# OSU-NLP-Group/saev

Hardware: AMD Instinct MI355X
Metric: activations/sec (train step), d_in=1024 x32 k=32 (higher is better)
Workload: dtype f32 (encoder: fp16 MFMA first pass with a rigorous error margin, survivors recomputed exactly in fp32; all else fp32)

## Files before the change

### saev_amd/csrc/ctx.hip

```cpp
#include <hip/hip_runtime.h>

#include <algorithm>
#include <cmath>
#include <cstdio>
#include <cstdlib>
#include <cstring>
#include <dlfcn.h>
#include <mutex>
#include <string>
#include <vector>

#include "kernels.h"

namespace {
constexpr int AUX_KSPLIT_MAX = 16;
constexpr int CAND_CAP = 4096;
constexpr int CAND_STRIDE = CAND_CAP + 256;
constexpr int TIMING_RING = 512;
constexpr int DEAD_LAG = 4;
constexpr int DEAD_RING = 16;
enum { AUX_NONE = 0, AUX_SMALL_DEVICE = 1, AUX_SMALL_HOST = 2, AUX_DENSE = 3 };
}

struct saev_ctx {
// ... 54 lines not shown
    bool dws_ok = false;
    int dws_rows = 0;
    bool dws_pairs = false;
    float *gS = nullptr, *xS = nullptr, *dvp = nullptr;
    float* xS_ov = nullptr;
    float* xS_bwd = nullptr;
    float* dval_rows = nullptr;
    bool dval_fwd = false;
    float* wn2 = nullptr;
    float* sq_wave = nullptr;
    int sq_wave_n = 0;
    bool wn2_fresh = false;
    float* WdS = nullptr;
    double* dec_part = nullptr;
    bool wds_fresh = false;
    bool dval_pairs_ready = false;
    bool fused_forward = false;
    bool fwd_slices = false;
    bool fwd_step = false;
    float* rs_part = nullptr;
    float* xS_c = nullptr;
    int2 *pv = nullptr, *pv2 = nullptr;
    int32_t *plat = nullptr, *cut_lat = nullptr, *cut_list = nullptr;
    int32_t* lat_unused = nullptr;
    bool fused_step = false;
    bool unused_valid = false;
    int P = 1;
    int32_t cuts[MAX_PREFIXES] = {0};
    float* G = nullptr;
    float* GS = nullptr;
    int P_cap = 0;
    int n_dead_host = 0, k_use_host = 0;
    int64_t tokens_seen = 0;
    bool tracker_dirty = false;
    int nd_cap = 0;
    DeadRecord* rec_host = nullptr;
    DeadRecord* rec_dev = nullptr;
    hipEvent_t dead_ev[DEAD_RING];
    bool dead_ev_created = false;
    int64_t dead_steps = 0;
    int64_t rec_valid_from = 1;
    int aux_route = AUX_NONE;
    int64_t n_readbacks = 0;
    std::vector<void*> aux_allocs;
    int32_t* dead_list = nullptr;
    float *Wenc_dead = nullptr, *Wdec_dead = nullptr, *H_dead = nullptr, *A_dead = nullptr, *dWd = nullptr, *dWe = nullptr,
// ... 231 lines not shown
    A(chunk_starts, S + 1); A(part_starts, S); A(work_latent, c->max_work);
    A(dW_encT, S * D); A(partials, (size_t)c->max_part * 2 * D); A(db_partials, c->max_part); A(row_proj, S); A(enc_sq, S);
    {
        const bool rows_only = c->dbg.dw_route == 1;
        c->dws_ok = !rows_only && D % DWS_SLICE == 0 && (uint64_t)S * D * 4ull < (1ull << 32) && MBB < (1l << 24) &&
                    (uint64_t)MBB * K < (1ull << 31);
    }
    c->fwd_slices = c->cfg.encoder_mode == SAEV_ENCODER_F16R && (c->dbg.fwd_route == 0 || c->dbg.fwd_route == 2) && c->dbg.fused_chain == 0 && D % RS_SLICE == 0 &&
                    (uint64_t)S * 128ull < (1ull << 32) - 256ull && fused_supported(c->cfg);
    if (c->fwd_slices) {
        A(rs_part, (size_t)(D / RS_SLICE) * MB * REFINE_CAP); A(surv_rng, MB * RS_MAX_RANGES);
        c->rs_lat_range = (int)std::max<long>(RS_LAT_RANGE, ((S + RS_MAX_RANGES - 1) / RS_MAX_RANGES + 255) / 256 * 256);
        c->rs_n_ranges = (int)((S + c->rs_lat_range - 1) / c->rs_lat_range);
    }
    if (c->fwd_slices && !c->dws_ok) A(xS, MBB * D);
    if (c->dws_ok) {
        A(gS, MBB * D); A(xS, MBB * D); A(dvp, (size_t)(D / DWS_SLICE) * MBB * K);
        if (c->dbg.dw_route != 2 && decode_forms_dval((int)D, (int)K)) A(dval_rows, MB * K);
        if (c->dval_rows != nullptr && c->dbg.dw_route == 4 && decode_slices_supported((int)D, (int)S, (int)K, (int)K) && c->cfg.normalize_w_dec) {
            A(WdS, S * D); A(dec_part, (size_t)(D / 32) * MB * 3);
        }
        A(pv, MBB * K); A(pv2, MBB * K); A(plat, MBB * K); A(cut_lat, (MBB * K + DWS_RUN - 1) / DWS_RUN); A(cut_list, 4 * (1 + (MBB * K + DWS_RUN - 1) / DWS_RUN)); A(lat_unused, S);
        if (c->dval_rows != nullptr && c->dbg.fin_route == 0) { A(wn2, S); A(sq_wave, (size_t)2 * dw_slices_waves((int)D, (int)(MBB * K))); }
    }
    A(colsum_partials, ((MBB + 63) / 64) * D);
    A(sumsq_partials, 2 * 1024 + (S + 3) / 4 + 8 + transpose_blocks((int)S, (int)D)); A(sumsq_total, 1);
    if (c->cfg.encoder_mode != SAEV_ENCODER_F32 || KA > 0) {
        c->Dp = (int)((D + 31) / 32 * 32);
        c->S_pad = (int)((S + 255) / 256 * 256);
        c->MB_pad = (int)((MB + 255) / 256 * 256);
        A(zero_bias, std::max(S, D)); A(aux_scales, 16); A(aux_sync, absmax_parts_max((int)MB));
    }
    if (c->cfg.encoder_mode != SAEV_ENCODER_F32) {
        A(xs, (size_t)c->MB_pad * 2 * c->Dp);
        A(ws, (size_t)c->S_pad * 2 * c->Dp);
        A(row_margin, MB); A(wnorm_scratch, std::max((S + 3) / 4, 3 * ((S + 255) / 256))); A(f16r_scales, 16); A(mu, D); A(xnorm, 2 * MB); A(b_shift, S);
        A(xabs_part, (MB + 3) / 4);
        if (c->cfg.encoder_mode == SAEV_ENCODER_F16R) { A(dot_part, (size_t)2 * (c->Dp / 32) * c->S_pad); A(sq_part, (size_t)2 * (c->Dp / 32) * c->S_pad); A(wmax_prev, 1); }
        if (c->cfg.encoder_mode == SAEV_ENCODER_F16R) { A(surv_idx, MB * REFINE_CAP); A(surv_val, MB * REFINE_CAP); A(surv_cnt, MB); }
    }
    c->stream_ok = c->fwd_slices && c->cfg.bound_mode == 0 && c->dbg.prep_route == 0 && D % 32 == 0 && c->Dp == (int)D;
    if (c->stream_ok) {
        A(WeS, S * D); A(xn_part, (size_t)(D / 32) * c->MB_pad * 2);
        A(amax_part, (size_t)(c->MB_pad / 256) * (D / 32)); A(cmax_part, (size_t)(c->MB_pad / 256) * (D / 32)); A(b_seen, S);
        A(mu_keep, D); A(xside_keep, 4);
    }
// ... 756 lines not shown
            HIPCHK(c, launch_normalize_rows(c->params + c->off_W_dec, S, D, s, c->WdS, c->wn2));
            c->wds_fresh = true;
            c->wn2_fresh = c->wn2 != nullptr;
        } else if (c->cfg.normalize_w_dec) {
            HIPCHK(c, launch_normalize_rows(c->params + c->off_W_dec, S, D, s, nullptr, c->wn2));
            c->wn2_fresh = c->wn2 != nullptr;
        }
    }

    DecodeArgs a{};
    a.x = x; a.idx = c->idx; a.val = c->val; a.code_stride = K; a.k = K;
    a.W_dec = c->params + c->off_W_dec; a.b_dec = c->params + c->off_b_dec;
    a.n_rows = n; a.D = D; a.S = S; a.idx_limit = S;
    a.upper = c->upper_c;
    a.gscale = 2.0f / ((float)n * (float)D * (float)c->P);
    a.training = training ? 1 : 0;
    a.g = c->g; a.x_hat = c->x_hat; a.fired = c->fired; a.rowstats = c->rowstats;
    c->dws_rows = 0;
    c->dval_fwd = false;
    if (training && c->dws_ok && (c->P == 1 || c->GS != nullptr)) { a.gS = c->P == 1 ? c->gS : c->GS; a.xS = c->fwd_step ? nullptr : c->xS; c->dws_rows = n; }
    if (c->dws_rows == n && c->dval_rows != nullptr && (c->P == 1 || decode_matry_forms_dval(D, K))) { a.dval_out = c->dval_rows; c->dval_fwd = true; }
    c->bitmap_prefill_words = 0;
    const bool slices_decode = c->P == 1 && c->wds_fresh && a.dval_out != nullptr && a.gS != nullptr;
    if (training && c->dbg.csc_route == 0 && c->bitmap != nullptr && c->bitmap_clean && !c->last_backward_gathered && !slices_decode) {
        const int words = ((n + 31) / 32 + 7) / 8 * 8;
        if (words <= c->bitmap_clean_words) {
            a.csc_bitmap = c->bitmap; a.csc_words = words;
            c->bitmap_prefill_words = words; c->bitmap_prefill_rows = n;
            c->bitmap_clean = false;
        }
    }
    if (slices_decode) {
        DecodeSliceArgs ds{};
        ds.d = a; ds.WdS = c->WdS; ds.part = c->dec_part; ds.dvp = c->dvp; ds.dvp_pitch = (long)c->back_rows * K;
        HIPCHK(c, launch_decode_slices(ds, s));
    } else if (c->P > 1) {
        MatryArgs m{};
        m.P = c->P;
        for (int p = 0; p < c->P; ++p) m.cuts[p] = c->cuts[p];
        m.G = c->G;
        m.g_rows_all = c->fused_forward ? 0 : 1;
        HIPCHK(c, launch_decode_matry(a, m, s));
    } else {
        HIPCHK(c, launch_decode(a, s));
    }
    c->P_last = c->P;
    for (int p = 0; p < c->P; ++p) c->cuts_last[p] = c->cuts[p];
// ... 389 lines not shown
    c->dws_pairs = ov ? ov_slices : c->dws_rows == n;
    if (ov_slices) {
        c->xS_bwd = c->xS;
        if (!c->followers.empty()) {
            if (c->xS_ov == nullptr) {
                int rca = alloc(c, &c->xS_ov, (size_t)c->back_rows * D);
                if (rca != SAEV_OK) return rca;
            }
            c->xS_bwd = c->xS_ov;
        }
        HIPCHK(c, launch_slice_major_copy(c->ov_g, c->ov_x, n, D, c->gS, c->xS_bwd, s));
        c->dws_rows = 0;
    }
    c->csc_epoch = c->csc_epoch == 0x7fffffff ? 1 : c->csc_epoch + 1;
    a.epoch = c->dbg.csc_route == 2 ? 0 : c->csc_epoch;
    if (c->dws_pairs) {
        a.zero_word = c->cut_list;
        a.pv = c->pv; a.plat = c->plat; a.val = ov ? c->ov_val : c->val;
        a.P = c->P_last;
        for (int p = 0; p < c->P_last; ++p) a.cuts[p] = c->cuts_last[p];
        if (!ov && c->dval_fwd) { a.pv2 = c->pv2; a.dval = c->dval_rows; }
    }
    c->dval_pairs_ready = c->dws_pairs && a.pv2 != nullptr;
    if (c->fused_step && c->dws_pairs) { a.pairs = nullptr; a.chunk_starts = nullptr; a.part_starts = nullptr; a.work_latent = nullptr; }
    const float* gmat = ov ? c->ov_g : (c->P_last > 1 ? c->G : c->g);
    const bool prefilled = !ov && c->bitmap_prefill_words == words && c->bitmap_prefill_rows == n;
    HIPCHK(c, launch_csc_build(a, s, c->bitmap_clean && words <= c->bitmap_clean_words, gmat, D, (long)c->P_last * D,
                               c->colsum_partials, c->grads + c->off_b_dec, prefilled));
    c->bitmap_prefill_words = 0;
    c->last_backward_gathered = ov;
    c->bitmap_clean = false;
    c->bitmap_words_last = words;
    if (c->aux_route != AUX_NONE) {
        int rc = auxk_backward(c, s);
        if (rc != SAEV_OK) return rc;
    }
    return SAEV_OK;
}

int saev_backward_rows(saev_ctx* c, int32_t lat_lo, int32_t lat_hi, void* stream) {
    return saev_backward_rows_part(c, lat_lo, lat_hi, 0, stream);
}

int saev_backward_rows_part(saev_ctx* c, int32_t lat_lo, int32_t lat_hi, int32_t part, void* stream) {
    if (!c) return SAEV_INVALID_ARG;
    REQUIRE(c, part >= 0 && part <= 2, SAEV_INVALID_ARG, "saev_backward_rows_part: part must be 0 (both), 1 (decoder) or 2 (encoder)");
// ... 15 lines not shown
    a.partials = c->partials; a.db_partials = c->db_partials;
    a.lat_lo = lat_lo; a.lat_hi = lat_hi;
    a.part = part; a.dval = c->dval_pairs;
    const bool all_rows = part == 0 && lat_lo == 0 && lat_hi == S;
    const bool clears = part != 2 && lat_lo == 0 && lat_hi == S && c->bitmap_words_last > 0;
    if (clears) { a.clear_bitmap = c->bitmap; a.clear_words = c->bitmap_words_last; }
    a.row_proj = all_rows ? c->row_proj : nullptr; a.project = c->cfg.remove_parallel_grads ? 1 : 0;
    a.enc_sq = all_rows ? c->enc_sq : nullptr;
    const int max_work = (lat_hi - lat_lo) + (int)(((long)n * K + DW_CHUNK - 1) / DW_CHUNK);
    if (lat_lo == 0 && lat_hi == S && c->dws_pairs && (ov || c->dws_rows == n)) {
        DwSlicesArgs w{};
        w.starts = c->starts; w.pv = c->pv; w.pv2 = c->pv2; w.plat = c->plat; w.gS = c->P_last > 1 ? c->GS : c->gS; w.W_dec = a.W_dec; w.P = c->P_last;
        w.xS = ov ? c->xS_bwd : (c->fwd_step ? c->xS_c : c->xS);
        w.n_rows = n; w.D = D; w.S = S; w.pair_cap = (int)((long)c->back_rows * K);
        w.dvp = c->dvp; w.dW_dec = a.dW_dec; w.dW_encT = a.dW_encT; w.db_enc = a.db_enc;
        const size_t runs_cap = ((size_t)w.pair_cap + DWS_RUN - 1) / DWS_RUN;
        w.part_dec = c->partials; w.part_enc = c->partials + 2 * runs_cap * D;
        w.cut_lat = c->cut_lat; w.cut_list = c->cut_list;
        w.lat_unused = (all_rows && c->fused_step) ? c->lat_unused : nullptr;
        c->unused_valid = w.lat_unused != nullptr;
        w.row_proj = a.row_proj; w.project = a.project; w.enc_sq = a.enc_sq;
        w.clear_bitmap = a.clear_bitmap; w.clear_words = a.clear_words;
        w.have_dval = c->dval_pairs_ready ? 1 : 0;
        c->sq_wave_n = 0;
        if (c->dval_pairs_ready && c->wn2_fresh && part == 0) {
            w.wn2 = c->wn2;
            if (c->fused_step && all_rows && c->sq_wave != nullptr && c->dbg.fin_route != 2) {
                c->sq_wave_n = dw_slices_waves(D, (int)((long)n * K));
                w.sq_wave_dec = c->sq_wave; w.sq_wave_enc = c->sq_wave + c->sq_wave_n;
            }
        }
        HIPCHK(c, launch_dw_slices(w, (int)((long)n * K), part, s));
    } else {
        c->unused_valid = false;
        HIPCHK(c, launch_dw_rows(a, max_work, s));
    }
    if (c->aux_route == AUX_DENSE)
        HIPCHK(c, launch_scatter_add_dead(c->dead_list, c->n_dead_host, D, c->dWd, c->dWe, c->dbe, c->grads + c->off_W_dec,
                                          c->dW_encT, c->grads + c->off_b_enc, lat_lo, lat_hi, s,
                                          c->aux_dev_count ? c->flags + 4 : nullptr, part, a.row_proj, a.W_dec, a.project, a.enc_sq,
                                          c->unused_valid ? c->lat_unused : nullptr, c->sq_wave_n > 0 ? c->starts : nullptr));
    else if (c->aux_route != AUX_NONE)
        HIPCHK(c, launch_scatter_add_dead(c->dead_list, c->aux_mfma ? c->aux_ndp : AUX_SMALL_MAX, D, c->dWd, c->dWe, c->dbe, c->grads + c->off_W_dec,
                                          c->dW_encT, c->grads + c->off_b_enc, lat_lo, lat_hi, s, c->flags + 4, part,
                                          a.row_proj, a.W_dec, a.project, a.enc_sq, c->unused_valid ? c->lat_unused : nullptr,
                                          c->sq_wave_n > 0 ? c->starts : nullptr));
// ... 540 lines not shown
```

### saev_amd/csrc/kernels.h

```cpp
#pragma once
#include <hip/hip_runtime.h>
#include <stdint.h>

#include "../../include/saev_amd.h"

enum { EPI_DENSE = 0, EPI_TOPK = 1 };

struct EncodeArgs {
    const float* x;
    const float* W_enc;
    const float* b_enc;
    int n_rows, D, S;
    int s_splits;
    float* h_out;
    int ngroups;
    int32_t* gmax;
    int gmax_stride;
    int32_t* cand_cnt;
    float* cand_val;
    int32_t* cand_idx;
    int cand_cap;
    int cand_stride;
    const int32_t* enable_flag;
    int enable_when;
// ... 139 lines not shown

struct CscArgs {
    const int32_t* idx;
    int code_stride, k;
    const int32_t* k_dev;
    int n_rows, S;
    uint32_t* bitmap;
    int words;
    int32_t* grp_prefix;
    int32_t* counts;
    int32_t* scan_totals;
    int32_t* starts;
    int2* pairs;
    int32_t* chunk_starts;
    int32_t* part_starts;
    int32_t* work_latent;
    int2* pv;
    int32_t* plat;
    const float* val;
    int2* pv2;
    const float* dval;
    int P;
    int32_t cuts[16];
    int32_t* zero_word;
    int32_t epoch;
};
hipError_t launch_csc_build(const CscArgs& a, hipStream_t stream, bool bitmap_clean = false, const float* colsum_m = nullptr,
                            int colsum_D = 0, long colsum_row_stride = 0, float* colsum_partials = nullptr,
                            float* colsum_out = nullptr, bool prefilled = false);

constexpr int DW_CHUNK = 64;

struct DwRowsArgs {
    const int32_t* starts;
    const int32_t* chunk_starts;
    const int32_t* work_latent;
    const int32_t* part_starts;
    const int2* pairs;
    const float* val;
    const float* W_dec;
    const float* g;
    const float* x;
    int D, S;
    int P;
    int32_t cuts[MAX_PREFIXES];
    const int32_t* k_dev;
// ... 24 lines not shown
    const float* gS;
    const float* xS;
    const float* W_dec;
    int n_rows, D, S, pair_cap;
    int P;
    float* dvp;
    float* dW_dec;
    float* dW_encT;
    float* db_enc;
    float* part_dec;
    float* part_enc;
    int32_t* cut_lat;
    int32_t* cut_list;
    float2* row_proj;
    int project;
    float* enc_sq;
    uint32_t* clear_bitmap;
    int clear_words;
    int32_t* lat_unused;
    int have_dval;
    const float* wn2;
    float* sq_wave_dec;
    float* sq_wave_enc;
};
hipError_t launch_dw_slices(const DwSlicesArgs& a, int max_pairs, int part, hipStream_t stream);
int dw_slices_waves(int D, int max_pairs);
hipError_t launch_slice_major_copy(const float* g, const float* x, int n, int D, float* gS, float* xS, hipStream_t stream);
hipError_t launch_transpose(const float* in, float* out, int S, int D, hipStream_t stream, double* sq_part = nullptr);
int transpose_blocks(int S, int D);

hipError_t launch_colsum(const float* m, int n_rows, int D, float* partials, float* out, int accumulate,
                         const int32_t* k_dev, hipStream_t stream, long row_stride = 0, float out_scale = 1.0f,
                         int col_mult = 0);
hipError_t launch_colsum_absmax(const float* m, int n_rows, int D, float* partials, float* out, float* wg_scratch,
                                float* absmax_out, hipStream_t stream, float out_scale = 1.0f,
                                saev_step_stats* zero_stats = nullptr, int32_t* zero_flag = nullptr);

hipError_t launch_normalize_rows(float* W, int S, int D, hipStream_t stream, float* WS = nullptr, float* wn2 = nullptr);
hipError_t launch_rpg(float* gW, const float* W, int S, int D, hipStream_t stream, double* sq_partials = nullptr,
                      int project = 1);
int sumsq_blocks();
hipError_t launch_sumsq_partials(const float* g, long n, double* partials, hipStream_t stream);
hipError_t launch_sumsq_final(const double* partials, int nb, double* total, hipStream_t stream);
hipError_t launch_sumsq(const float* g, long n, double* partials, double* total, hipStream_t stream);
struct AdamArgs {
    float* p; const float* g; float* m; float* v;
// ... 289 lines not shown
```

### saev_amd/csrc/select.hip

```cpp
#include "common.h"
#include "kernels.h"

namespace {

constexpr int SD_THREADS = 256;

__device__ __forceinline__ int block_excl_scan_256(int v, int* lds_wave_tot, int& total) {
    const int lane = threadIdx.x & 63, w = threadIdx.x >> 6;
    int incl = v;
#pragma unroll
    for (int o = 1; o < 64; o <<= 1) {
        int n = __shfl_up(incl, o, 64);
        if (lane >= o) incl += n;
    }
    if (lane == 63) lds_wave_tot[w] = incl;
    __syncthreads();
    int base = 0, tot = 0;
#pragma unroll
    for (int i = 0; i < 4; ++i) {
        const int t = lds_wave_tot[i];
        if (i < w) base += t;
        tot += t;
    }
    total = tot;
    __syncthreads();
    return base + incl - v;
}

__global__ __launch_bounds__(SD_THREADS) void select_dense_kernel(SelectDenseArgs a) {
    if (a.enable_flag != nullptr && (*a.enable_flag != 0) != (a.enable_when != 0)) return;
    __shared__ int hist[256];
    __shared__ int sh_digit, sh_need;
    __shared__ int wave_tot[4];

    const int row = blockIdx.x;
    const int S = a.S;
    int k = a.k_dev ? min(*a.k_dev, a.k) : a.k;
    if (a.k_dev && k <= 0) return;
    const float* h = a.h + (size_t)row * S;
    const int tid = threadIdx.x;
    const int S4 = S >> 2;

    uint32_t prefix = 0, pmask = 0;
    int need = k;

    for (int pass = 0; pass < 4; ++pass) {
        const int shift = 24 - 8 * pass;
        hist[tid] = 0;
        __syncthreads();
        for (int q = tid; q < S4; q += SD_THREADS) {
            const f32x4 v = *reinterpret_cast<const f32x4*>(h + 4 * q);
            int4 mk = {1, 1, 1, 1};
            if (a.mask) mk = *reinterpret_cast<const int4*>(a.mask + 4 * q);
            const int m[4] = {mk.x, mk.y, mk.z, mk.w};
#pragma unroll
            for (int e = 0; e < 4; ++e) {
                const uint32_t key = f2ukey(v[e]);
                if (m[e] != 0 && (key & pmask) == prefix) atomicAdd(&hist[(key >> shift) & 255], 1);
// ... 53 lines not shown
        const int neq = feq[0] + feq[1] + feq[2] + feq[3];
        int tot;
        const int ex = block_excl_scan_256(ngt | (neq << 16), wave_tot, tot);
        int gt_before = base_gt + (ex & 0xFFFF);
        int eq_before = base_eq + (ex >> 16);
#pragma unroll
        for (int e = 0; e < 4; ++e) {
            if (flg[e]) {
                const int pos = gt_before + min(eq_before, need);
                oi[pos] = 4 * q + e;
                ov[pos] = v[e];
                ++gt_before;
            } else if (feq[e]) {
                if (eq_before < need) {
                    const int pos = gt_before + eq_before;
                    oi[pos] = 4 * q + e;
                    ov[pos] = v[e];
                }
                ++eq_before;
            }
        }
        base_gt += tot & 0xFFFF;
        base_eq += tot >> 16;
    }
}


__device__ __forceinline__ float wave_reduce_scatter8(float (&p)[8], int lane) {
    int bit = 32;
#pragma unroll
    for (int h = 4; h >= 1; h >>= 1, bit >>= 1) {
        const bool up = (lane & bit) != 0;
#pragma unroll
        for (int i = 0; i < h; ++i) {
            const float keep = up ? p[i + h] : p[i];
            const float send = up ? p[i] : p[i + h];
            p[i] = keep + __shfl_xor(send, bit, 64);
        }
    }
    float r = p[0];
    for (; bit >= 1; bit >>= 1) r += __shfl_xor(r, bit, 64);
    return r;
}

__device__ __forceinline__ void sort_by_idx_and_store(const SelectCandArgs& a, int row, int k, int32_t my_idx, float my_val,
                                                      int lane) {
// ... 855 lines not shown
    if (state[5] > 0.f) { state[5] -= 1.f; g = 1; }
    *gate = g;
}
__global__ void heur_update_kernel(float* state, const int32_t* bad, const float* cand_mean, int k, const int32_t* gate) {
    if (threadIdx.x != 0 || *gate != 0) return;
    float z = state[0];
    state[2] += 1.f;
    if (*bad != 0) {
        z -= 0.3f;
        state[1] += 1.f;
        state[4] += 1.f;
        if (state[4] >= 3.f) { state[4] = 0.f; state[5] = 256.f; z = 1.5f; }
    } else {
        state[4] = 0.f;
        if (*cand_mean > 3.f * (float)k) z += 0.002f;
    }
    state[0] = fminf(fmaxf(z, 0.5f), 3.5f);
}

}

hipError_t launch_select_dense(const SelectDenseArgs& a, hipStream_t stream) {
    if (a.n_rows <= 0) return hipSuccess;
    hipLaunchKernelGGL(select_dense_kernel, dim3(a.n_rows), dim3(SD_THREADS), 0, stream, a);
    return hipGetLastError();
}

hipError_t launch_select_cand(const SelectCandArgs& a, hipStream_t stream) {
    if (a.n_rows <= 0) return hipSuccess;
    if (a.cand_cap > 4096 || (a.sum_part != nullptr && a.cand_cap > REFINE_CAP)) return hipErrorInvalidValue;
    if (a.k > 32) hipLaunchKernelGGL(select_cand_kernel<true>, dim3((a.n_rows + 3) / 4), dim3(256), 0, stream, a);
    else hipLaunchKernelGGL(select_cand_kernel<false>, dim3((a.n_rows + 3) / 4), dim3(256), 0, stream, a);
    return hipGetLastError();
}

hipError_t launch_init_i32(int32_t* p, int32_t v, int n, hipStream_t stream) {
    if (n <= 0) return hipSuccess;
    hipLaunchKernelGGL(init_i32_kernel, dim3((n + 255) / 256), dim3(256), 0, stream, p, v, n);
    return hipGetLastError();
}

hipError_t launch_encoder_init(int32_t* cand_cnt, int n_rows, int32_t* gmax, int n_gmax, hipStream_t stream, int32_t* tau_max,
                               const int32_t* enable_flag, int enable_when) {
    const int n = n_rows > n_gmax ? n_rows : n_gmax;
    if (n <= 0) return hipSuccess;
    hipLaunchKernelGGL(encoder_init_kernel, dim3((n + 255) / 256), dim3(256), 0, stream, cand_cnt, n_rows, gmax, n_gmax, tau_max,
                       enable_flag, enable_when);
// ... 110 lines not shown
```

### saev_amd/csrc/sparse.hip

```cpp
#include "common.h"
#include "kernels.h"

namespace {

template <int NV>
__device__ __forceinline__ void gather_rows_accum(f32x4 (&acc)[NV], const float* __restrict__ W, int D, int D4,
                                                  const int32_t* idx_row, const float* val_row, int k, int limit,
                                                  int lane) {
    for (int j0 = 0; j0 < k; j0 += 64) {
        const int cnt = min(64, k - j0);
        int32_t my_i = -1;
        float my_v = 0.f;
        if (lane < cnt) { my_i = idx_row[j0 + lane]; my_v = val_row[j0 + lane]; }
#pragma unroll 4
        for (int jj = 0; jj < cnt; ++jj) {
            const int32_t i = __shfl(my_i, jj, 64);
            const float v = __shfl(my_v, jj, 64);
            if (i < 0 || i >= limit) continue;
            const f32x4* wr = reinterpret_cast<const f32x4*>(W + (size_t)i * D);
#pragma unroll
            for (int n = 0; n < NV; ++n) {
                const int q = lane + 64 * n;
                if (q < D4) {
                    const f32x4 w = wr[q];
                    acc[n] += v * w;
                }
// ... 584 lines not shown
    const long n = (long)a.n_rows * k;
    const int groups = a.words >> 3;
    for (long p = (long)blockIdx.x * blockDim.x + threadIdx.x; p < max(n, (long)a.S); p += (long)gridDim.x * blockDim.x) {
        if (p < a.S && a.chunk_starts) {
            const int c1 = a.chunk_starts[p + 1];
            for (int c = a.chunk_starts[p]; c < c1; ++c) a.work_latent[c] = (int)p;
        }
        if (p >= n) continue;
        const int b = (int)(p / k), j = (int)(p % k);
        const int32_t i = a.idx[(size_t)b * a.code_stride + j];
        if (i < 0 || i >= a.S) continue;
        const int g = b >> 8, wi = (b >> 5) & 7;
        const uint4* grp = reinterpret_cast<const uint4*>(a.bitmap + (size_t)i * a.words + 8 * g);
        const uint4 lo = grp[0], hi = grp[1];
        const uint32_t wd[8] = {lo.x, lo.y, lo.z, lo.w, hi.x, hi.y, hi.z, hi.w};
        int rank = a.grp_prefix[(size_t)i * groups + g];
#pragma unroll
        for (int e = 0; e < 8; ++e) {
            const uint32_t m = e < wi ? 0xffffffffu : (e == wi ? ((1u << (b & 31)) - 1u) : 0u);
            rank += __popc(wd[e] & m);
        }
        const int slot = a.starts[i] + rank;
        if (a.pairs != nullptr) a.pairs[slot] = int2{b, (int)((size_t)b * a.code_stride + j)};
        if (a.pv != nullptr) {
            const int fl = (rank == 0 ? DWS_FIRST : 0) | (rank == a.counts[i] - 1 ? DWS_LAST : 0);
            int pblk = 0;
            if (a.P > 1) while (pblk < a.P - 1 && i >= a.cuts[pblk]) ++pblk;
            a.pv[slot] = int2{((pblk * a.n_rows + b) << 7) | fl, __float_as_int(a.val[(size_t)b * a.code_stride + j])};
            a.plat[slot] = i;
            if (a.pv2 != nullptr) a.pv2[slot] = int2{(b << 7) | fl, __float_as_int(a.dval[(size_t)b * a.code_stride + j])};
        }
    }
}


template <int NV>
__device__ __forceinline__ void write_row_proj(float2* row_proj, int i, const f32x4 (&g)[NV], const f32x4 (&w)[NV], int project,
                                               int lane) {
    float sc;
    const float sq = rpg_row_stats<NV>(g, w, project, &sc);
    if (lane == 0) row_proj[i] = float2{sc, sq};
}

template <int NV>
__device__ __forceinline__ float row_sumsq(const f32x4 (&g)[NV]) {
    float sq = 0.f;
#pragma unroll
// ... 189 lines not shown
    }
    f32x4* o = reinterpret_cast<f32x4*>((enc ? a.dW_encT : a.dW_dec) + (size_t)i * D);
#pragma unroll
    for (int n = 0; n < NV; ++n) {
        const int q = lane + 64 * n;
        if (q < D4) o[q] = a.accumulate ? o[q] + acc[n] : acc[n];
    }
    if (enc) {
        if (lane == 0) a.db_enc[i] = a.accumulate ? (a.db_enc[i] + dbs) : dbs;
        if (a.enc_sq != nullptr && !a.accumulate) {
            const float sq = row_sumsq<NV>(acc);
            if (lane == 0) a.enc_sq[i] = sq;
        }
    } else if (a.row_proj != nullptr && !a.accumulate) {
        f32x4 wv[NV];
        const f32x4* wr = reinterpret_cast<const f32x4*>(a.W_dec + (size_t)i * D);
#pragma unroll
        for (int n = 0; n < NV; ++n) wv[n] = (lane + 64 * n < D4) ? wr[lane + 64 * n] : f32x4{0.f, 0.f, 0.f, 0.f};
        write_row_proj<NV>(a.row_proj, i, acc, wv, a.project, lane);
    }
}


typedef int i32x2 __attribute__((ext_vector_type(2)));
typedef int i32x4 __attribute__((ext_vector_type(4)));

__device__ __forceinline__ f32x4 buf_load16(__amdgpu_buffer_rsrc_t r, uint32_t voff) {
    const i32x4 v = __builtin_amdgcn_raw_buffer_load_b128(r, voff, 0, 0);
    return f32x4{__int_as_float(v[0]), __int_as_float(v[1]), __int_as_float(v[2]), __int_as_float(v[3])};
}
__device__ __forceinline__ float group8_sum(float v) {
    v += __int_as_float(__builtin_amdgcn_mov_dpp(__float_as_int(v), 0xB1, 0xF, 0xF, true));
    v += __int_as_float(__builtin_amdgcn_mov_dpp(__float_as_int(v), 0x4E, 0xF, 0xF, true));
    v += __int_as_float(__builtin_amdgcn_mov_dpp(__float_as_int(v), 0x141, 0xF, 0xF, true));
    return v;
}

__global__ __launch_bounds__(256) void slice_major_copy_kernel(const float* __restrict__ g, const float* __restrict__ x, int n, int D,
                                                               float* __restrict__ gS, float* __restrict__ xS) {
    const int lane = threadIdx.x & 63;
    const int row = blockIdx.x * 4 + (threadIdx.x >> 6);
    if (row >= n) return;
    const f32x4* gr = reinterpret_cast<const f32x4*>(g + (size_t)row * D);
    const f32x4* xr = reinterpret_cast<const f32x4*>(x + (size_t)row * D);
    for (int q = lane; q < (D >> 2); q += 64) {
        const size_t o = ((size_t)(q >> 3) * n + row) * 8 + (q & 7);
        reinterpret_cast<f32x4*>(gS)[o] = gr[q];
        reinterpret_cast<f32x4*>(xS)[o] = xr[q];
    }
}

template <bool DEC, bool DVAL = true>
__global__ __launch_bounds__(256, (DEC && DVAL) ? 4 : 5) void dw_slices_kernel(DwSlicesArgs a, int wg_per_slice) {
    constexpr bool PASS_A = DEC && DVAL;
    constexpr int L = DWS_RUN;
    const int lane = threadIdx.x & 63, gi = lane >> 3, li = lane & 7;
    const int xcd = blockIdx.x & 7, q = blockIdx.x >> 3;
    const int slice = xcd + 8 * (q / wg_per_slice);
    const bool sq_on = (DEC ? a.sq_wave_dec : a.sq_wave_enc) != nullptr;
    auto sq_slot = [&]() -> float* {
        return (DEC ? a.sq_wave_dec : a.sq_wave_enc) + ((size_t)blockIdx.x * 4 + __builtin_amdgcn_readfirstlane((int)(threadIdx.x >> 6)));
    };
    if (slice * DWS_SLICE >= a.D) { if (sq_on && lane == 0) *sq_slot() = 0.f; return; }
    const int NP = a.starts[a.S];
    const int run0 = ((q % wg_per_slice) * 4 + (threadIdx.x >> 6)) * 8;
    if (run0 * L >= NP) { if (sq_on && lane == 0) *sq_slot() = 0.f; return; }
    const int run = run0 + gi;
    const int col = slice * DWS_SLICE + li * 4;
    const uint32_t colb = (uint32_t)col * 4u, rowb = (uint32_t)a.D * 4u, li16 = (uint32_t)li * 16u;
    auto bound = [&](int r) -> int {
        const long nb = (long)r * L;
        if (nb >= NP) return NP;
        const int lat = a.plat[nb];
        const int s = a.starts[lat];
        return (a.starts[lat + 1] - s < L) ? s : (int)nb;
    };
    const int p0 = bound(run), p1 = bound(run + 1);
    const bool live = p0 < p1;
    const int2* const pv = DEC ? a.pv : a.pv2;
    float* const out = DEC ? a.dW_dec : a.dW_encT;
    float* const part = DEC ? a.part_dec : a.part_enc;
    f32x4 acc = {0.f, 0.f, 0.f, 0.f};
    f32x4 w4 = {0.f, 0.f, 0.f, 0.f};
    float* const dvp = PASS_A ? a.dvp + (size_t)slice * a.pair_cap : nullptr;
    __shared__ float sh_sq[256];
    sh_sq[threadIdx.x] = 0.f;
    const int sel = (lane & 56) << 2;
    const __amdgpu_buffer_rsrc_t mres = __builtin_amdgcn_make_buffer_rsrc(
        const_cast<float*>(DEC ? a.gS : a.xS) + (size_t)slice * a.n_rows * DWS_SLICE * (DEC && a.P > 1 ? a.P : 1), 0,
        (uint32_t)a.n_rows * 128u * (uint32_t)(DEC && a.P > 1 ? a.P : 1), 0x00020000);
    const __amdgpu_buffer_rsrc_t wres = __builtin_amdgcn_make_buffer_rsrc(const_cast<float*>(a.W_dec), 0, (uint32_t)a.S * rowb, 0x00020000);

    auto load_info = [&](int t, int2& e, int& lat) {
        const int p = p0 + 8 * t + li;
        e = int2{0, 0};
        lat = 0;
        if (p < p1) {
            const i32x2 v = reinterpret_cast<const i32x2*>(pv)[p];
            e = int2{v[0], v[1]};
            lat = a.plat[p];
            if (p == p1 - 1) e.x |= DWS_END;
            if (p == p0) e.x &= ~DWS_FIRST;
        }
    };
    constexpr int PB = 4;
    auto issue = [&](const int2& e, int lat, int j0, int (&xj)[PB], int (&lj)[PB], f32x4 (&gt)[PB], f32x4 (&wt)[PB]) {
#pragma unroll
        for (int j = 0; j < PB; ++j) {
            xj[j] = __builtin_amdgcn_ds_bpermute(sel + 4 * (j0 + j), e.x);
            lj[j] = __builtin_amdgcn_ds_bpermute(sel + 4 * (j0 + j), lat);
            gt[j] = buf_load16(mres, ((uint32_t)xj[j] & ~127u) | li16);
            if (PASS_A && (xj[j] & DWS_FIRST)) wt[j] = buf_load16(wres, (uint32_t)lj[j] * rowb + colb);
        }
    };
    auto consume = [&](const int2& e, int j0, const int (&xc)[PB], const int (&lc)[PB], const f32x4 (&gc)[PB], const f32x4 (&wc)[PB],
                       const f32x4& wnext0, bool& head_open, float& dmine) {
        float vc[PB];
#pragma unroll
        for (int j = 0; j < PB; ++j) vc[j] = __int_as_float(__builtin_amdgcn_ds_bpermute(sel + 4 * (j0 + j), e.y));
#pragma unroll
        for (int j = 0; j < PB; ++j) {
            if (PASS_A) {
                float d = gc[j][0] * w4[0] + gc[j][1] * w4[1] + gc[j][2] * w4[2] + gc[j][3] * w4[3];
// ... 10 lines not shown
                    if (sq_on)
                        sh_sq[threadIdx.x] += __builtin_fmaf(acc[3], acc[3], __builtin_fmaf(acc[2], acc[2], __builtin_fmaf(acc[1], acc[1], acc[0] * acc[0])));
                }
                *reinterpret_cast<f32x4*>(o) = acc;
                if (DEC && slice == 0 && li == 0 && (xc[j] & DWS_END)) {
                    const int cl = (!head_open && !(xc[j] & DWS_LAST)) ? lc[j] : -1;
                    a.cut_lat[run] = cl;
                    if (cl >= 0 && a.cut_list != nullptr)
                        reinterpret_cast<i32x4*>(a.cut_list)[1 + atomicAdd(&a.cut_list[0], 1)] = i32x4{run, cl, a.starts[cl], a.starts[cl + 1]};
                }
                head_open = false;
                acc = f32x4{0.f, 0.f, 0.f, 0.f};
                if (PASS_A) w4 = j + 1 < PB ? wc[j + 1 < PB ? j + 1 : 0] : wnext0;
            }
        }
    };
    int2 e_c, e_n;
    int lat_c, lat_n;
    int xa[PB], xb[PB], la[PB], lb[PB];
    f32x4 ga[PB], gb[PB], wa[PB], wb[PB];
    bool head_open = false;
    load_info(0, e_c, lat_c);
    if (live) {
        head_open = (pv[p0].x & DWS_FIRST) == 0;
        if (PASS_A) w4 = buf_load16(wres, (uint32_t)a.plat[p0] * rowb + colb);
    }
    issue(e_c, lat_c, 0, xa, la, ga, wa);
    load_info(1, e_n, lat_n);
#pragma unroll 1
    for (int t = 0; __any(p0 + 8 * t < p1); ++t) {
        float dmine = 0.f;
        issue(e_c, lat_c, PB, xb, lb, gb, wb);
        consume(e_c, 0, xa, la, ga, wa, wb[0], head_open, dmine);
        issue(e_n, lat_n, 0, xa, la, ga, wa);
        consume(e_c, PB, xb, lb, gb, wb, wa[0], head_open, dmine);
        if (PASS_A && p0 + 8 * t + li < p1) dvp[p0 + 8 * t + li] = dmine;
        e_c = e_n; lat_c = lat_n;
        load_info(t + 2, e_n, lat_n);
    }
    if (sq_on) {
        const float sq = wave_sum(sh_sq[threadIdx.x]);
        if (lane == 0) *sq_slot() = sq;
    }
}

__global__ __launch_bounds__(256) void dw_dval_sum_kernel(DwSlicesArgs a) {
    const int NP = a.starts[a.S];
// ... 125 lines not shown
    for (int n = 0; n < NV; ++n) {
        acc[n] = f32x4{0.f, 0.f, 0.f, 0.f};
        wv[n] = f32x4{0.f, 0.f, 0.f, 0.f};
        if (lane + 64 * n < D4) {
            if (e > s) acc[n] = reinterpret_cast<const f32x4*>(row)[lane + 64 * n];
            else if (!(enc && a.lat_unused != nullptr)) reinterpret_cast<f32x4*>(row)[lane + 64 * n] = acc[n];
            if (proj) wv[n] = wr[lane + 64 * n];
        }
    }
    if (enc) {
        float dbs = 0.f;
        for (int p = s + lane; p < e; p += 64) dbs += __int_as_float(a.pv2[p].y);
        dbs = wave_sum(dbs);
        if (lane == 0) a.db_enc[i] = dbs;
        if (a.enc_sq != nullptr) {
            const float sq = row_sumsq<NV>(acc);
            if (lane == 0) a.enc_sq[i] = sq;
        }
    } else if (proj) {
        write_row_proj<NV>(a.row_proj, i, acc, wv, a.project, lane);
    }
}

template <int NV>
__global__ __launch_bounds__(256) void dw_finalize_light_kernel(DwSlicesArgs a, int n_cut_blocks) {
    constexpr int L = DWS_RUN;
    __shared__ f32x4 sh[3][NV * 64];
    __shared__ float shdb[4];
    const int lane = threadIdx.x & 63, w = threadIdx.x >> 6;
    const int D = a.D, D4 = D >> 2;
    if ((int)blockIdx.x < n_cut_blocks) {
      const i32x4 first = reinterpret_cast<const i32x4*>(a.cut_list)[1 + (blockIdx.x >> 1)];
      const int n_items = 2 * a.cut_list[0];
      for (int item = blockIdx.x; item < n_items; item += n_cut_blocks) {
        const i32x4 ent = item == (int)blockIdx.x ? first : reinterpret_cast<const i32x4*>(a.cut_list)[1 + (item >> 1)];
        const int r0 = ent[0], i = ent[1], s = ent[2], e = ent[3], enc = item & 1;
        const int r1 = (e - 1) / L;
        const float* const part = enc ? a.part_enc : a.part_dec;
        f32x4 tp[NV], wv[NV];
        if (w == 0) {
            const f32x4* p = reinterpret_cast<const f32x4*>(part + ((size_t)r0 * 2 + 1) * D);
            const f32x4* wr = reinterpret_cast<const f32x4*>(a.W_dec + (size_t)i * D);
            const bool need_w = !enc && a.row_proj != nullptr;
#pragma unroll
            for (int n = 0; n < NV; ++n) {
                const bool ok = lane + 64 * n < D4;
                tp[n] = ok ? p[lane + 64 * n] : f32x4{0.f, 0.f, 0.f, 0.f};
                wv[n] = (ok && need_w) ? wr[lane + 64 * n] : f32x4{0.f, 0.f, 0.f, 0.f};
            }
// ... 31 lines not shown
                const f32x4* p = reinterpret_cast<const f32x4*>(part + (size_t)(r + u) * 2 * D);
#pragma unroll
                for (int n = 0; n < NV; ++n) t[u][n] = (lane + 64 * n < D4) ? p[lane + 64 * n] : f32x4{0.f, 0.f, 0.f, 0.f};
            }
#pragma unroll
            for (int n = 0; n < NV; ++n) {
                if constexpr (TRIP == 4) acc[n] += (t[0][n] + t[1][n]) + (t[2][n] + t[3][n]);
                else acc[n] += t[0][n] + t[1][n];
            }
        }
        for (; r < rb; ++r) {
            const f32x4* p = reinterpret_cast<const f32x4*>(part + (size_t)r * 2 * D);
#pragma unroll
            for (int n = 0; n < NV; ++n)
                if (lane + 64 * n < D4) acc[n] += p[lane + 64 * n];
        }
        float dbs = 0.f;
        if (enc) {
            const int cnt = e - s, q4 = (cnt + 3) / 4;
            const int pend = min(e, s + (w + 1) * q4);
            for (int p0 = s + w * q4 + lane; p0 < pend; p0 += 64 * 8) {
                int2 pe[8];
#pragma unroll
                for (int u = 0; u < 8; ++u) pe[u] = (p0 + 64 * u < pend) ? a.pv2[p0 + 64 * u] : int2{0, 0};
#pragma unroll
                for (int u = 0; u < 8; ++u) {
                    if (p0 + 64 * u < pend) {
                        dbs += __int_as_float(pe[u].y);
                        if (a.clear_bitmap != nullptr) a.clear_bitmap[(size_t)i * a.clear_words + (pe[u].x >> 12)] = 0u;
                    }
                }
            }
            dbs = wave_sum(dbs);
        }
        if (w != 0) {
#pragma unroll
            for (int n = 0; n < NV; ++n) sh[w - 1][lane + 64 * n] = acc[n];
        }
        if (lane == 0) shdb[w] = dbs;
        __syncthreads();
        if (w == 0) {
#pragma unroll
            for (int n = 0; n < NV; ++n) acc[n] = (((tp[n] + acc[n]) + sh[0][lane + 64 * n]) + sh[1][lane + 64 * n]) + sh[2][lane + 64 * n];
            float* const row = (enc ? a.dW_encT : a.dW_dec) + (size_t)i * D;
#pragma unroll
            for (int n = 0; n < NV; ++n)
                if (lane + 64 * n < D4) reinterpret_cast<f32x4*>(row)[lane + 64 * n] = acc[n];
// ... 40 lines not shown
    };
    float gsq = 0.f, esq = 0.f;
    const bool waves_hold_squares = a.sq_wave_dec != nullptr;
    if (!waves_hold_squares) {
        const f32x4* gd = reinterpret_cast<const f32x4*>(a.dW_dec + (size_t)i * D);
        const f32x4* ge = reinterpret_cast<const f32x4*>(a.dW_encT + (size_t)i * D);
#pragma unroll 4
        for (int q = li; q < D4; q += 8) {
            const f32x4 u = gd[q], v = ge[q];
            gsq = __builtin_fmaf(u[3], u[3], __builtin_fmaf(u[2], u[2], __builtin_fmaf(u[1], u[1], __builtin_fmaf(u[0], u[0], gsq))));
            esq = __builtin_fmaf(v[3], v[3], __builtin_fmaf(v[2], v[2], __builtin_fmaf(v[1], v[1], __builtin_fmaf(v[0], v[0], esq))));
        }
        gsq += __shfl_xor(gsq, 4, 64); gsq += __shfl_xor(gsq, 2, 64); gsq += __shfl_xor(gsq, 1, 64);
        esq += __shfl_xor(esq, 4, 64); esq += __shfl_xor(esq, 2, 64); esq += __shfl_xor(esq, 1, 64);
    }
    float dv8[8], dt8[8];
#pragma unroll
    for (int j = 0; j < 8; ++j) {
        float dbs = 0.f, dot = 0.f;
#pragma unroll
        for (int t = 0; t < 2; ++t) {
            const int p = s + li + 8 * j + 64 * t;
            if (p < e) {
                const int2 pd = a.pv2[p];
                const float dv = __int_as_float(pd.y);
                dbs += dv;
                dot = __builtin_fmaf(__int_as_float(a.pv[p].y), dv, dot);
                if (a.clear_bitmap != nullptr) a.clear_bitmap[(size_t)i * a.clear_words + (pd.x >> 12)] = 0u;
            }
        }
        dv8[j] = dbs; dt8[j] = dot;
    }
    const float dbs = group_tree(dv8), dot = group_tree(dt8);
    if (li == 0) {
        a.db_enc[i] = dbs;
        if (a.enc_sq != nullptr) a.enc_sq[i] = esq;
        if (a.row_proj != nullptr) {
            const float nsq = a.wn2[i];
            const float sc = (a.project && nsq > 0.f) ? dot / nsq : 0.f;
            a.row_proj[i] = float2{sc, waves_hold_squares ? -sc * dot : fmaxf(__builtin_fmaf(-sc, dot, gsq), 0.f)};
        }
    }
}

__global__ __launch_bounds__(256) void transpose_kernel(const float* __restrict__ in, float* __restrict__ out, int S,
                                                        int D, double* __restrict__ sq_part) {
    __shared__ float tile[64][65];
    __shared__ double sh[4];
    const int s0 = blockIdx.x * 64, d0 = blockIdx.y * 64;
    const int c4 = (threadIdx.x & 15) * 4, r0 = threadIdx.x >> 4;
// ... 490 lines not shown
hipError_t launch_dw_rows(const DwRowsArgs& a, int max_work, hipStream_t stream) {
    return dispatch_nv(a.D, [&](auto nv) {
        hipLaunchKernelGGL(dw_rows_kernel<decltype(nv)::value>, dim3((max_work + 3) / 4), dim3(256), 0, stream, a);
        hipLaunchKernelGGL(dw_combine_kernel<decltype(nv)::value>, dim3((a.lat_hi - a.lat_lo + 3) / 4, 2), dim3(256), 0, stream, a);
    });
}
hipError_t launch_slice_major_copy(const float* g, const float* x, int n, int D, float* gS, float* xS, hipStream_t stream) {
    if (n <= 0) return hipSuccess;
    hipLaunchKernelGGL(slice_major_copy_kernel, dim3((n + 3) / 4), dim3(256), 0, stream, g, x, n, D, gS, xS);
    return hipGetLastError();
}
int dw_slices_waves(int D, int max_pairs) {
    const int n_runs = (max_pairs + DWS_RUN - 1) / DWS_RUN;
    return ((D / DWS_SLICE + 7) / 8) * 8 * ((n_runs + 31) / 32) * 4;
}
hipError_t launch_dw_slices(const DwSlicesArgs& a_in, int max_pairs, int part, hipStream_t stream) {
    DwSlicesArgs a = a_in;
    if (a.D % DWS_SLICE != 0 || max_pairs <= 0) return hipErrorInvalidValue;
    const int n_runs = (max_pairs + DWS_RUN - 1) / DWS_RUN;
    const int wg_per_slice = (n_runs + 31) / 32;
    const int grid = ((a.D / DWS_SLICE + 7) / 8) * 8 * wg_per_slice;
    const bool light = part == 0 && a.have_dval && a.wn2 != nullptr;
    if (!light) { a.sq_wave_dec = nullptr; a.sq_wave_enc = nullptr; }
    if (part != 2 && a.have_dval) {
        hipLaunchKernelGGL((dw_slices_kernel<true, false>), dim3(grid), dim3(256), 0, stream, a, wg_per_slice);
        if (a.clear_bitmap != nullptr && !light) hipLaunchKernelGGL(dw_clear_bitmap_kernel, dim3((max_pairs + 255) / 256), dim3(256), 0, stream, a);
    } else if (part != 2) {
        hipLaunchKernelGGL(dw_slices_kernel<true>, dim3(grid), dim3(256), 0, stream, a, wg_per_slice);
        hipLaunchKernelGGL(dw_dval_sum_kernel, dim3((max_pairs + 255) / 256), dim3(256), 0, stream, a);
    }
    if (part != 1) hipLaunchKernelGGL(dw_slices_kernel<false>, dim3(grid), dim3(256), 0, stream, a, wg_per_slice);
    const int kinds = part == 0 ? 2 : 1, kind0 = part == 2 ? 1 : 0;
    if (light) {
        const int n_cut = a.cut_list != nullptr ? std::min(2 * (n_runs - 1), 8192) : 0;
        if (a.cut_list == nullptr && n_runs > 1) return hipErrorInvalidValue;
        return dispatch_nv(a.D, [&](auto nv) {
            hipLaunchKernelGGL(dw_finalize_light_kernel<decltype(nv)::value>, dim3(n_cut + (a.S + 31) / 32), dim3(256), 0, stream, a, n_cut);
        });
    }
    return dispatch_nv(a.D, [&](auto nv) {
        if (n_runs > 1) hipLaunchKernelGGL(dw_finalize_cut_kernel<decltype(nv)::value>, dim3(n_runs - 1, kinds), dim3(256), 0, stream, a, kind0);
        hipLaunchKernelGGL(dw_finalize_kernel<decltype(nv)::value>, dim3((a.S + 3) / 4, kinds), dim3(256), 0, stream, a, kind0);
    });
}
hipError_t launch_transpose(const float* in, float* out, int S, int D, hipStream_t stream, double* sq_part) {
    hipLaunchKernelGGL(transpose_kernel, dim3((S + 63) / 64, (D + 63) / 64), dim3(256), 0, stream, in, out, S, D, sq_part);
    return hipGetLastError();
}
int transpose_blocks(int S, int D) { return ((S + 63) / 64) * ((D + 63) / 64); }
hipError_t launch_colsum(const float* m, int n_rows, int D, float* partials, float* out, int accumulate,
                         const int32_t* k_dev, hipStream_t stream, long row_stride, float out_scale, int col_mult) {
    const int nb = (n_rows + 63) / 64;
    if (nb <= 0) return hipSuccess;
    hipLaunchKernelGGL(colsum_partial_kernel<false>, dim3(nb), dim3(256), 0, stream, m, n_rows, D, partials, k_dev,
                       row_stride > 0 ? row_stride : (long)D, (float*)nullptr, col_mult);
    hipLaunchKernelGGL(colsum_final_kernel, dim3((D + 63) / 64), dim3(256), 0, stream, partials, nb, D, out,
                       accumulate, k_dev, out_scale, col_mult, (const float*)nullptr, (float*)nullptr, (saev_step_stats*)nullptr,
                       (int32_t*)nullptr);
    return hipGetLastError();
}
// ... 12 lines not shown
```

Before: 6.242 million.

## Pack sparse pair records into int4 and grid-stride predicated dense select

Result: faster. 6.329 million, median of 6 (+1.4%).

```diff
diff --git a/saev_amd/csrc/ctx.hip b/saev_amd/csrc/ctx.hip
--- a/saev_amd/csrc/ctx.hip
+++ b/saev_amd/csrc/ctx.hip
@@ -100,6 +100,8 @@
     float* xS_c = nullptr;
     int2 *pv = nullptr, *pv2 = nullptr;
     int32_t *plat = nullptr, *cut_lat = nullptr, *cut_list = nullptr;
+    int4* prec = nullptr;
+    bool pairs_packed = false;
     int32_t* lat_unused = nullptr;
     bool fused_step = false;
     bool unused_valid = false;
@@ -377,6 +379,7 @@
         }
         A(pv, MBB * K); A(pv2, MBB * K); A(plat, MBB * K); A(cut_lat, (MBB * K + DWS_RUN - 1) / DWS_RUN); A(cut_list, 4 * (1 + (MBB * K + DWS_RUN - 1) / DWS_RUN)); A(lat_unused, S);
         if (c->dval_rows != nullptr && c->dbg.fin_route == 0) { A(wn2, S); A(sq_wave, (size_t)2 * dw_slices_waves((int)D, (int)(MBB * K))); }
+        if (c->wn2 != nullptr && c->dbg.csc_route != 3) A(prec, MBB * K);
     }
     A(colsum_partials, ((MBB + 63) / 64) * D);
     A(sumsq_partials, 2 * 1024 + (S + 3) / 4 + 8 + transpose_blocks((int)S, (int)D)); A(sumsq_total, 1);
@@ -1179,7 +1182,7 @@
     if (c->dws_rows == n && c->dval_rows != nullptr && (c->P == 1 || decode_matry_forms_dval(D, K))) { a.dval_out = c->dval_rows; c->dval_fwd = true; }
     c->bitmap_prefill_words = 0;
     const bool slices_decode = c->P == 1 && c->wds_fresh && a.dval_out != nullptr && a.gS != nullptr;
-    if (training && c->dbg.csc_route == 0 && c->bitmap != nullptr && c->bitmap_clean && !c->last_backward_gathered && !slices_decode) {
+    if (training && (c->dbg.csc_route == 0 || c->dbg.csc_route == 3) && c->bitmap != nullptr && c->bitmap_clean && !c->last_backward_gathered && !slices_decode) {
         const int words = ((n + 31) / 32 + 7) / 8 * 8;
         if (words <= c->bitmap_clean_words) {
             a.csc_bitmap = c->bitmap; a.csc_words = words;
@@ -1615,6 +1618,8 @@
         if (!ov && c->dval_fwd) { a.pv2 = c->pv2; a.dval = c->dval_rows; }
     }
     c->dval_pairs_ready = c->dws_pairs && a.pv2 != nullptr;
+    c->pairs_packed = c->dval_pairs_ready && c->fused_step && c->P_last <= 1 && c->wn2_fresh && c->prec != nullptr;
+    if (c->pairs_packed) { a.prec = c->prec; a.pv = nullptr; a.pv2 = nullptr; a.plat = nullptr; }
     if (c->fused_step && c->dws_pairs) { a.pairs = nullptr; a.chunk_starts = nullptr; a.part_starts = nullptr; a.work_latent = nullptr; }
     const float* gmat = ov ? c->ov_g : (c->P_last > 1 ? c->G : c->g);
     const bool prefilled = !ov && c->bitmap_prefill_words == words && c->bitmap_prefill_rows == n;
@@ -1676,6 +1681,7 @@
         w.row_proj = a.row_proj; w.project = a.project; w.enc_sq = a.enc_sq;
         w.clear_bitmap = a.clear_bitmap; w.clear_words = a.clear_words;
         w.have_dval = c->dval_pairs_ready ? 1 : 0;
+        w.prec = c->pairs_packed ? c->prec : nullptr;
         c->sq_wave_n = 0;
         if (c->dval_pairs_ready && c->wn2_fresh && part == 0) {
             w.wn2 = c->wn2;
diff --git a/saev_amd/csrc/kernels.h b/saev_amd/csrc/kernels.h
--- a/saev_amd/csrc/kernels.h
+++ b/saev_amd/csrc/kernels.h
@@ -185,6 +185,7 @@
     const float* dval;
     int P;
     int32_t cuts[16];
+    int4* prec;
     int32_t* zero_word;
     int32_t epoch;
 };
@@ -255,6 +256,7 @@
     const float* wn2;
     float* sq_wave_dec;
     float* sq_wave_enc;
+    const int4* prec;
 };
 hipError_t launch_dw_slices(const DwSlicesArgs& a, int max_pairs, int part, hipStream_t stream);
 int dw_slices_waves(int D, int max_pairs);
diff --git a/saev_amd/csrc/select.hip b/saev_amd/csrc/select.hip
--- a/saev_amd/csrc/select.hip
+++ b/saev_amd/csrc/select.hip
@@ -27,13 +27,11 @@
     return base + incl - v;
 }
 
-__global__ __launch_bounds__(SD_THREADS) void select_dense_kernel(SelectDenseArgs a) {
-    if (a.enable_flag != nullptr && (*a.enable_flag != 0) != (a.enable_when != 0)) return;
+__device__ __forceinline__ void select_dense_row(const SelectDenseArgs& a, int row) {
     __shared__ int hist[256];
     __shared__ int sh_digit, sh_need;
     __shared__ int wave_tot[4];
 
-    const int row = blockIdx.x;
     const int S = a.S;
     int k = a.k_dev ? min(*a.k_dev, a.k) : a.k;
     if (a.k_dev && k <= 0) return;
@@ -133,6 +131,15 @@
         }
         base_gt += tot & 0xFFFF;
         base_eq += tot >> 16;
+    }
+}
+
+constexpr int SD_PRED_WGS = 1024;
+__global__ __launch_bounds__(SD_THREADS) void select_dense_kernel(SelectDenseArgs a) {
+    if (a.enable_flag != nullptr && (*a.enable_flag != 0) != (a.enable_when != 0)) return;
+    for (int row = blockIdx.x; row < a.n_rows; row += gridDim.x) {
+        select_dense_row(a, row);
+        __syncthreads();
     }
 }
 
@@ -1034,7 +1041,8 @@
 
 hipError_t launch_select_dense(const SelectDenseArgs& a, hipStream_t stream) {
     if (a.n_rows <= 0) return hipSuccess;
-    hipLaunchKernelGGL(select_dense_kernel, dim3(a.n_rows), dim3(SD_THREADS), 0, stream, a);
+    const int grid = a.enable_flag != nullptr ? std::min(a.n_rows, SD_PRED_WGS) : a.n_rows;
+    hipLaunchKernelGGL(select_dense_kernel, dim3(grid), dim3(SD_THREADS), 0, stream, a);
     return hipGetLastError();
 }
 
diff --git a/saev_amd/csrc/sparse.hip b/saev_amd/csrc/sparse.hip
--- a/saev_amd/csrc/sparse.hip
+++ b/saev_amd/csrc/sparse.hip
@@ -2,6 +2,9 @@
 #include "kernels.h"
 
 namespace {
+
+typedef int i32x2 __attribute__((ext_vector_type(2)));
+typedef int i32x4 __attribute__((ext_vector_type(4)));
 
 template <int NV>
 __device__ __forceinline__ void gather_rows_accum(f32x4 (&acc)[NV], const float* __restrict__ W, int D, int D4,
@@ -632,7 +635,11 @@
         }
         const int slot = a.starts[i] + rank;
         if (a.pairs != nullptr) a.pairs[slot] = int2{b, (int)((size_t)b * a.code_stride + j)};
-        if (a.pv != nullptr) {
+        if (a.prec != nullptr) {
+            const int fl = (rank == 0 ? DWS_FIRST : 0) | (rank == a.counts[i] - 1 ? DWS_LAST : 0);
+            const size_t o = (size_t)b * a.code_stride + j;
+            reinterpret_cast<i32x4*>(a.prec)[slot] = i32x4{(b << 7) | fl, __float_as_int(a.dval[o]), __float_as_int(a.val[o]), i};
+        } else if (a.pv != nullptr) {
             const int fl = (rank == 0 ? DWS_FIRST : 0) | (rank == a.counts[i] - 1 ? DWS_LAST : 0);
             int pblk = 0;
             if (a.P > 1) while (pblk < a.P - 1 && i >= a.cuts[pblk]) ++pblk;
@@ -868,9 +875,6 @@
 }
 
 
-typedef int i32x2 __attribute__((ext_vector_type(2)));
-typedef int i32x4 __attribute__((ext_vector_type(4)));
-
 __device__ __forceinline__ f32x4 buf_load16(__amdgpu_buffer_rsrc_t r, uint32_t voff) {
     const i32x4 v = __builtin_amdgcn_raw_buffer_load_b128(r, voff, 0, 0);
     return f32x4{__int_as_float(v[0]), __int_as_float(v[1]), __int_as_float(v[2]), __int_as_float(v[3])};
@@ -896,9 +900,11 @@
     }
 }
 
-template <bool DEC, bool DVAL = true>
+template <bool DEC, bool DVAL = true, bool PK = false>
 __global__ __launch_bounds__(256, (DEC && DVAL) ? 4 : 5) void dw_slices_kernel(DwSlicesArgs a, int wg_per_slice) {
     constexpr bool PASS_A = DEC && DVAL;
+    static_assert(!(PK && PASS_A), "the records carry dval: pass A never forms it from them");
+    const i32x4* const rec = reinterpret_cast<const i32x4*>(a.prec);
     constexpr int L = DWS_RUN;
     const int lane = threadIdx.x & 63, gi = lane >> 3, li = lane & 7;
     const int xcd = blockIdx.x & 7, q = blockIdx.x >> 3;
@@ -917,7 +923,7 @@
     auto bound = [&](int r) -> int {
         const long nb = (long)r * L;
         if (nb >= NP) return NP;
-        const int lat = a.plat[nb];
+        const int lat = PK ? reinterpret_cast<const int32_t*>(a.prec)[4 * nb + 3] : a.plat[nb];
         const int s = a.starts[lat];
         return (a.starts[lat + 1] - s < L) ? s : (int)nb;
     };
@@ -942,9 +948,15 @@
         e = int2{0, 0};
         lat = 0;
         if (p < p1) {
-            const i32x2 v = reinterpret_cast<const i32x2*>(pv)[p];
-            e = int2{v[0], v[1]};
-            lat = a.plat[p];
+            if (PK) {
+                const i32x4 v = rec[p];
+                e = int2{v[0], DEC ? v[2] : v[1]};
+                lat = v[3];
+            } else {
+                const i32x2 v = reinterpret_cast<const i32x2*>(pv)[p];
+                e = int2{v[0], v[1]};
+                lat = a.plat[p];
+            }
             if (p == p1 - 1) e.x |= DWS_END;
             if (p == p0) e.x &= ~DWS_FIRST;
         }
@@ -1001,7 +1013,7 @@
     bool head_open = false;
     load_info(0, e_c, lat_c);
     if (live) {
-        head_open = (pv[p0].x & DWS_FIRST) == 0;
+        head_open = ((PK ? reinterpret_cast<const int32_t*>(a.prec)[4 * (size_t)p0] : pv[p0].x) & DWS_FIRST) == 0;
         if (PASS_A) w4 = buf_load16(wres, (uint32_t)a.plat[p0] * rowb + colb);
     }
     issue(e_c, lat_c, 0, xa, la, ga, wa);
@@ -1173,9 +1185,13 @@
     }
 }
 
-template <int NV>
+template <int NV, bool PK>
 __global__ __launch_bounds__(256) void dw_finalize_light_kernel(DwSlicesArgs a, int n_cut_blocks) {
     constexpr int L = DWS_RUN;
+    const i32x4* const rec = reinterpret_cast<const i32x4*>(a.prec);
+    auto pair_dval = [&](int p) -> int2 {
+        return PK ? reinterpret_cast<const int2*>(a.prec)[2 * (size_t)p] : a.pv2[p];
+    };
     __shared__ f32x4 sh[3][NV * 64];
     __shared__ float shdb[4];
     const int lane = threadIdx.x & 63, w = threadIdx.x >> 6;
@@ -1253,7 +1269,7 @@
             for (int p0 = s + w * q4 + lane; p0 < pend; p0 += 64 * 8) {
                 int2 pe[8];
 #pragma unroll
-                for (int u = 0; u < 8; ++u) pe[u] = (p0 + 64 * u < pend) ? a.pv2[p0 + 64 * u] : int2{0, 0};
+                for (int u = 0; u < 8; ++u) pe[u] = (p0 + 64 * u < pend) ? pair_dval(p0 + 64 * u) : int2{0, 0};
 #pragma unroll
                 for (int u = 0; u < 8; ++u) {
                     if (p0 + 64 * u < pend) {
@@ -1340,10 +1356,19 @@
         for (int t = 0; t < 2; ++t) {
             const int p = s + li + 8 * j + 64 * t;
             if (p < e) {
-                const int2 pd = a.pv2[p];
+                int2 pd;
+                float va;
+                if (PK) {
+                    const i32x4 v = rec[p];
+                    pd = int2{v[0], v[1]};
+                    va = __int_as_float(v[2]);
+                } else {
+                    pd = a.pv2[p];
+                    va = __int_as_float(a.pv[p].y);
+                }
                 const float dv = __int_as_float(pd.y);
                 dbs += dv;
-                dot = __builtin_fmaf(__int_as_float(a.pv[p].y), dv, dot);
+                dot = __builtin_fmaf(va, dv, dot);
                 if (a.clear_bitmap != nullptr) a.clear_bitmap[(size_t)i * a.clear_words + (pd.x >> 12)] = 0u;
             }
         }
@@ -1880,20 +1905,26 @@
     const int grid = ((a.D / DWS_SLICE + 7) / 8) * 8 * wg_per_slice;
     const bool light = part == 0 && a.have_dval && a.wn2 != nullptr;
     if (!light) { a.sq_wave_dec = nullptr; a.sq_wave_enc = nullptr; }
-    if (part != 2 && a.have_dval) {
+    const bool pk = a.prec != nullptr;
+    if (pk && !light) return hipErrorInvalidValue;
+    if (pk) {
+        hipLaunchKernelGGL((dw_slices_kernel<true, false, true>), dim3(grid), dim3(256), 0, stream, a, wg_per_slice);
+    } else if (part != 2 && a.have_dval) {
         hipLaunchKernelGGL((dw_slices_kernel<true, false>), dim3(grid), dim3(256), 0, stream, a, wg_per_slice);
         if (a.clear_bitmap != nullptr && !light) hipLaunchKernelGGL(dw_clear_bitmap_kernel, dim3((max_pairs + 255) / 256), dim3(256), 0, stream, a);
     } else if (part != 2) {
         hipLaunchKernelGGL(dw_slices_kernel<true>, dim3(grid), dim3(256), 0, stream, a, wg_per_slice);
         hipLaunchKernelGGL(dw_dval_sum_kernel, dim3((max_pairs + 255) / 256), dim3(256), 0, stream, a);
     }
-    if (part != 1) hipLaunchKernelGGL(dw_slices_kernel<false>, dim3(grid), dim3(256), 0, stream, a, wg_per_slice);
+    if (pk) hipLaunchKernelGGL((dw_slices_kernel<false, true, true>), dim3(grid), dim3(256), 0, stream, a, wg_per_slice);
+    else if (part != 1) hipLaunchKernelGGL(dw_slices_kernel<false>, dim3(grid), dim3(256), 0, stream, a, wg_per_slice);
     const int kinds = part == 0 ? 2 : 1, kind0 = part == 2 ? 1 : 0;
     if (light) {
         const int n_cut = a.cut_list != nullptr ? std::min(2 * (n_runs - 1), 8192) : 0;
         if (a.cut_list == nullptr && n_runs > 1) return hipErrorInvalidValue;
         return dispatch_nv(a.D, [&](auto nv) {
-            hipLaunchKernelGGL(dw_finalize_light_kernel<decltype(nv)::value>, dim3(n_cut + (a.S + 31) / 32), dim3(256), 0, stream, a, n_cut);
+            if (pk) hipLaunchKernelGGL((dw_finalize_light_kernel<decltype(nv)::value, true>), dim3(n_cut + (a.S + 31) / 32), dim3(256), 0, stream, a, n_cut);
+            else hipLaunchKernelGGL((dw_finalize_light_kernel<decltype(nv)::value, false>), dim3(n_cut + (a.S + 31) / 32), dim3(256), 0, stream, a, n_cut);
         });
     }
     return dispatch_nv(a.D, [&](auto nv) {
```
